# wmtlab/tactileSR

Hardware: AMD Instinct MI355X
Metric: SR samples/sec (4x4->40x40) (higher is better)
Workload: dtype f32 as 2 power-of-two-scaled fp16 planes x 3 MFMA products, fp32 accumulate (fp32-grade); 1 GPU; tactileSR_model eval forward 4x4->40x40, batch=4096/GPU, fp32 in/out (BASELINE configs[1]); batch_per_gpu=4096, scale_factor=10, seqsCnt=1, parallelism=replicas x1, conv_impl=fp16x3, dist_world_size=1

## Files before the change

### include/tactilesr_hip.h

```cpp
#ifndef TACTILESR_HIP_H
#define TACTILESR_HIP_H
#ifdef __cplusplus
extern "C" {
#endif

#define TSR_OK 0
#define TSR_ERR_ARG 1
#define TSR_ERR_LAUNCH 2

int tsr_abi_version(void);

int tsr_build_flags(void);

int tsr_pack_conv_weight(const float* w_oihw, float* w_packed, int cout, int cin, int ks, void* stream);

int tsr_conv2d_fwd(const float* in, int in_ctot, int in_coff, int cin,
                   const float* w_packed, int cout, int ks,
                   const float* scale, const float* shift,
                   const float* res, int res_ctot, int res_coff,
                   float* out, int out_ctot, int out_coff, int relu,
                   int B, int H, int W, void* stream);

long long tsr_conv_weight_bf16s_elems(int cout, int cin, int ks, int nsplit);
int tsr_pack_conv_weight_bf16s(const float* w_oihw, void* w_packed, int cout, int cin, int ks, int nsplit,
// ... 20 lines not shown
int tsr_conv2d_fwd_f16s(const float* in, int in_ctot, int in_coff, int cin,
                        const void* w_packed, int cout, int ks, float w_inv_scale,
                        const float* in_amax, float* out_amax,
                        const float* scale, const float* shift,
                        const float* res, int res_ctot, int res_coff,
                        float* out, int out_ctot, int out_coff, int relu,
                        int B, int H, int W, void* stream);
int tsr_conv2d_fwd_f16s_fuse1x1(const float* in, int in_ctot, int in_coff, int cin,
                                const void* w_packed, int ks, float w_inv_scale,
                                const float* in_amax, float* out_amax,
                                const float* scale, const float* shift, int relu,
                                const void* w2_packed, float w2_inv_scale, const float* shift2,
                                const float* res, int res_ctot, int res_coff,
                                float* out, int out_ctot, int out_coff, int relu2,
                                int B, int H, int W, void* stream);
int tsr_conv2d_fwd_b16(const void* in, int in_ctot, int in_coff, int cin, const void* w_packed, int cout, int ks,
                       const float* scale, const float* shift, const void* res, int res_ctot, int res_coff,
                       void* out, int out_ctot, int out_coff, int relu, int B, int H, int W, void* stream);
long long tsr_conv_weight_b16k_elems(int cout, int cin, int ks);
int tsr_pack_conv_weight_b16k(const float* w_oihw, void* w_packed, int cout, int cin, int ks, void* stream);
int tsr_pack_w2_b16k(const float* w2_64x128, void* w_packed, void* stream);
int tsr_conv2d_ex_dgrad_b16k(int nprime, int cout, int ks);
int tsr_conv2d_ex_fwd1x1_b16k(int cout, int cin);
int tsr_pack_conv_weight_dgrad_b16k(const float* w_oihw, void* w_packed, int cout, int cin, int ks, int ci0, int nprime,
                                    void* stream);
long long tsr_conv_weight_b16k_pair_elems(int cin);
int tsr_pack_conv_weight_b16k_pair(const float* w128_oihw5, void* w_packed, int cin, void* stream);
int tsr_conv2d_fwd_b16k(const void* in, int in_ctot, int in_coff, int cin, const void* w_packed, int cout, int ks,
                        const float* scale, const float* shift, const void* res, int res_ctot, int res_coff,
                        void* out, int out_ctot, int out_coff, int relu, int B, int H, int W, void* stream);
// ... 252 lines not shown
```

### tactilesr_amd/_lib.py

```python
from __future__ import annotations

import ctypes
import os
from ctypes import c_int, c_void_p, c_float, c_longlong, c_double

import torch

_HERE = os.path.dirname(os.path.abspath(__file__))
LIB_PATH = os.environ.get("TSR_LIB_OVERRIDE") or os.path.join(_HERE, "lib", "libtactilesr_hip.so")
ABI_VERSION = 24

_P, _I, _F, _L = c_void_p, c_int, c_float, c_longlong

SIGNATURES = {
    "tsr_abi_version": [],
    "tsr_build_flags": [],
    "tsr_pack_conv_weight": [_P, _P, _I, _I, _I, _P],
    "tsr_conv2d_fwd": [_P, _I, _I, _I, _P, _I, _I, _P, _P, _P, _I, _I, _P, _I, _I, _I, _I, _I, _I, _P],
    "tsr_conv_weight_bf16s_elems": [_I, _I, _I, _I],
    "tsr_pack_conv_weight_bf16s": [_P, _P, _I, _I, _I, _I, _P],
    "tsr_conv2d_fwd_bf16s": [_P, _I, _I, _I, _P, _I, _I, _I, _P, _P, _P, _I, _I, _P, _I, _I, _I, _I, _I, _I, _P],
    "tsr_stem_fwd": [_P, _I, _I, _I, _I, _I, _I, _P, _P, _P, _P, _I, _I, _I, _I, _P, _P],
    "tsr_pack_conv_weight_f16s": [_P, _P, _I, _I, _I, _F, _P],
    "tsr_pack_conv_weight_f16s_dev": [_P, _P, _I, _I, _I, _P, _P],
    "tsr_pack_conv_weight_dgrad_f16s_dev": [_P, _P, _I, _I, _I, _I, _I, _P, _P],
    "tsr_conv2d_fwd_f16s": [_P, _I, _I, _I, _P, _I, _I, _F, _P, _P, _P, _P, _P, _I, _I, _P, _I, _I, _I, _I, _I, _I, _P],
    "tsr_conv2d_fwd_f16s_fuse1x1": [_P, _I, _I, _I, _P, _I, _F, _P, _P, _P, _P, _I, _P, _F, _P, _P, _I, _I, _P, _I, _I,
                                    _I, _I, _I, _I, _P],
    "tsr_pair_channel_perm": [_P],
    "tsr_conv_weight_pair_elems": [_I],
    "tsr_pack_conv_weight_pair_f16s": [_P, _P, _P, _I, _F, _P, _P],
    "tsr_conv2d_fwd_f16s_pair": [_P, _I, _I, _I, _P, _F, _P, _P, _P, _P, _P, _I, _I, _I, _I, _I, _I, _P],
    "tsr_head_fwd": [_P, _I, _I, _P, _P, _I, _I, _I, _I, _P],
    "tsr_conv2d_fwd_b16": [_P, _I, _I, _I, _P, _I, _I, _P, _P, _P, _I, _I, _P, _I, _I, _I, _I, _I, _I, _P],
    "tsr_conv_weight_b16k_elems": [_I, _I, _I],
    "tsr_pack_conv_weight_b16k": [_P, _P, _I, _I, _I, _P],
    "tsr_pack_w2_b16k": [_P, _P, _P],
    "tsr_conv2d_ex_dgrad_b16k": [_I, _I, _I],
    "tsr_pack_conv_weight_dgrad_b16k": [_P, _P, _I, _I, _I, _I, _I, _P],
    "tsr_conv_weight_b16k_pair_elems": [_I],
    "tsr_pack_conv_weight_b16k_pair": [_P, _P, _I, _P],
    "tsr_conv2d_fwd_b16k": [_P, _I, _I, _I, _P, _I, _I, _P, _P, _P, _I, _I, _P, _I, _I, _I, _I, _I, _I, _P],
    "tsr_conv2d_fwd_b16k_fuse1x1": [_P, _I, _I, _I, _P, _I, _P, _P, _I, _P, _P, _P, _I, _I, _P, _I, _I, _I, _I, _I, _I, _P],
    "tsr_conv2d_fwd_b16k_pair": [_P, _I, _I, _I, _P, _P, _P, _P, _I, _I, _I, _I, _I, _I, _P],
    "tsr_stem_fwd_b16": [_P, _I, _I, _I, _I, _I, _I, _P, _P, _P, _P, _I, _I, _I, _I, _P],
    "tsr_head_fwd_b16": [_P, _I, _I, _P, _P, _I, _I, _I, _I, _P],
    "tsr_conv2d_ex": [_P, _P],
# ... 151 lines not shown
```

### tactilesr_amd/csrc/conv_args.h

```cpp
#pragma once
struct ConvArgs {
  const float* in;  int in_ctot;  int in_coff;  int cin;
  const float* wp;
  const float* scale; const float* shift;
  const float* res; int res_ctot; int res_coff;
  float* out; int out_ctot; int out_coff;
  int relu;
  int B, H, W;
  int tiles_x, tiles_y;
  const float* in_scale; const float* in_shift;
  const float* res_scale; const float* res_shift;
  int epi_mode;
  const float* mask; int mask_ctot; int mask_coff;
  const float* mask_scale; const float* mask_shift;
  const float* bn_a; const float* bn_b;
  float* slab; float* slab_cnt;
  const float* in_amax;
  float w_inv_scale;
  float* out_amax;
  const void* w2;
  float w2_inv_scale;
  const float* shift2;
  int relu2;
  const float* w_amax;
};
```

### tactilesr_amd/csrc/conv_epilogue16.h

```cpp
#pragma once
#include "tsr_common.h"
#include "conv_args.h"
#include "conv_epilogue.h"

template <int COUT, bool EXT, int WN = 2, bool IO16 = false>
__device__ __forceinline__ void conv_epilogue16(const ConvArgs& a, f32x4 (&acc)[4][COUT / (16 * WN)], int ebase, int b0,
                                                int y0, int x0, int wm, int wn, int lane, int HW, float accmul = 1.f) {
  constexpr int NT = COUT / (16 * WN);
  const int cl = lane & 15, ph = lane >> 4;
  const int k4 = cl >> 2, j = cl & 3;
  const int dyl = ph >> 1, dxl = 4 * (ph & 1);
  float amax = 0.f;
  const int b = b0 + wm;
  const bool img_ok = b < a.B;
  const int out_blocks = a.out_ctot >> 4;
  const int res_blocks = a.res_ctot >> 4;
  const int mask_blocks = a.mask_ctot >> 4;
  const int bsafe = img_ok ? b : 0;
  typedef __bf16 ep_bf16x4 __attribute__((ext_vector_type(4)));
  const int gx = x0 + dxl + j;
  const f32x4 one4v = {1.f, 1.f, 1.f, 1.f}, zero4v = {0.f, 0.f, 0.f, 0.f};
  f32x4 pv0[NT], pv1[NT], pv2[NT], pv3[NT], pv4[NT];
  const bool m2 = EXT && a.epi_mode == 2, m0 = !EXT || a.epi_mode == 0;
#pragma unroll
// ... 54 lines not shown
          for (int c = 0; c < 4; ++c) v[c] = (v[c] * accmul) * sc4[c] + sh4[c];
          if (rb4) {
            f32x4 rv = rvv[mt];
            if (EXT && a.res_scale) {
#pragma unroll
              for (int c = 0; c < 4; ++c) rv[c] = tsr_relu(fmaf(rv[c], rsc4[c], rsh4[c]));
            }
#pragma unroll
            for (int c = 0; c < 4; ++c) v[c] += rv[c];
          }
#pragma unroll
          for (int c = 0; c < 4; ++c) {
            if (a.relu) v[c] = tsr_relu(v[c]);
            amax = fmaxf(amax, fabsf(v[c]));
          }
          if (IO16) {
            ep_bf16x4 o16;
#pragma unroll
            for (int c = 0; c < 4; ++c) o16[c] = (__bf16)v[c];
            *(ep_bf16x4*)((__bf16*)a.out + oidx4 + po) = o16;
          } else {
            *(f32x4*)(ob4 + po) = v;
          }
        }
      }
    } else if (EXT && a.epi_mode == 1) {
      float cnt = 0.f, sum = 0.f;
#pragma unroll
      for (int mt = 0; mt < 4; ++mt) {
#pragma unroll
        for (int r = 0; r < 4; ++r) {
// ... 83 lines not shown
        for (int c = 0; c < 4; ++c) {
          s1[c] += __shfl_xor(s1[c], 1); s2[c] += __shfl_xor(s2[c], 1);
          s1[c] += __shfl_xor(s1[c], 2); s2[c] += __shfl_xor(s2[c], 2);
          s1[c] += __shfl_xor(s1[c], 16); s2[c] += __shfl_xor(s2[c], 16);
          s1[c] += __shfl_xor(s1[c], 32); s2[c] += __shfl_xor(s2[c], 32);
        }
        if (ph == 0 && j == 0) {
          const size_t e = (size_t)ebase + wm;
          float* sl = a.slab + (e * COUT + nq) * 2;
#pragma unroll
          for (int c = 0; c < 4; ++c) { sl[2 * c] = s1[c]; sl[2 * c + 1] = s2[c]; }
        }
      }
    }
  }
  if (a.out_amax) {
#pragma unroll
    for (int o = 32; o > 0; o >>= 1) amax = fmaxf(amax, __shfl_xor(amax, o));
    if (lane == 0) publish_amax(a.out_amax, amax);
  }
}
```

### tactilesr_amd/csrc/conv_mfma_k32.hip

```cpp
#include "tsr_common.h"
#include "conv_args.h"
#include "conv_epilogue16.h"
#include "conv_fuse1x1_16.h"
#include "conv_host.h"
#include "tactilesr_hip.h"
#include <type_traits>

typedef _Float16 kf16x8 __attribute__((ext_vector_type(8)));
typedef _Float16 kf16x4 __attribute__((ext_vector_type(4)));

constexpr int k32_row_slots(int px) {
  int rs = px * 4;
  while ((rs & 3) != 2) ++rs;
  return rs;
}

template <int KS, int COUT, int WN, bool DBH = false, int NTHR = 256> struct K32Geom {
  static constexpr int IMG = (NTHR / 64) / WN;
  static constexpr int HH = 8 + KS - 1;
  static constexpr int T = KS * KS;
  static constexpr int HS = (T - 1) / 2;
  static constexpr int PIXB = 64;
  static constexpr int ROWB = k32_row_slots(HH) * 16;
  static constexpr int IMGB = HH * ROWB;
  static constexpr int HALO_B = IMG * IMGB;
  static constexpr int SROWB = k32_row_slots(8) * 16;
  static constexpr int SIMGB = 8 * SROWB;
  static constexpr int SIDE_B = DBH ? 0 : IMG * SIMGB;
  static constexpr int WTAP_B = 2 * 16 * COUT * 2;
  static constexpr int WSLAB_B = 2 * WTAP_B;
  static constexpr int NHB = DBH ? 2 : 1;
  static constexpr int MAIN_LDS = NHB * HALO_B + SIDE_B + 3 * WSLAB_B;
};

constexpr int PAIR_KH[12] = {0, 0, 0, 2, 1, 3, 4, 4, 1, 1, 2, 3};
constexpr int PAIR_KW[12] = {0, 2, 4, 4, 0, 0, 1, 3, 1, 3, 1, 1};
constexpr int PAIR_V[12] = {0, 0, 1, 1, 1, 1, 0, 0, 0, 1, 0, 0};
constexpr int PAIR_OUTER = 8;

template <int KS, int COUT, bool EXT, int WN, bool FUSE2 = false, bool DBH = false, int NTHR = 256, bool PAIR = false>
__global__ __launch_bounds__(NTHR, NTHR == 512 ? 1 : 2) void conv_k32_kernel(const ConvArgs a) {
  static_assert(!PAIR || (KS == 5 && COUT == 128 && !EXT && !FUSE2 && !DBH), "pair form: 5x5 geometry, inference");
  static_assert(COUT == 64 * WN, "every wave owns 64 channels");
  static_assert(!FUSE2 || (!EXT && COUT == 128), "fused 1x1: 128 channels, inference");
  static_assert(NTHR == 256 || (NTHR == 512 && WN == 2), "512 threads: 4 images x 2 C_out halves");
  typedef K32Geom<KS, COUT, WN, DBH, NTHR> G;
  constexpr int NW = NTHR / 64;
  constexpr bool WDMA = !EXT;
  constexpr int IMG = G::IMG, P = KS / 2, HH = G::HH, T = G::T, HS = G::HS, NT = COUT / (16 * WN);
  constexpr int PIXB = G::PIXB, ROWB = G::ROWB, IMGB = G::IMGB, HALO_B = G::HALO_B;
  constexpr int SROWB = G::SROWB, SIMGB = G::SIMGB, SIDE_B = G::SIDE_B;
  constexpr int WTAP_B = G::WTAP_B, WSLAB_B = G::WSLAB_B;
  constexpr int WITEMS = WSLAB_B / 16, WV = (WITEMS + NTHR - 1) / NTHR;
  constexpr int NITEM = IMG * HH * HH * 4, NIT = (NITEM + NTHR - 1) / NTHR;
  constexpr int FUSE_LDS = FUSE2 ? Fuse1x1Geom16<IMG>::BYTES + 64 : 0;
  __shared__ __attribute__((aligned(16))) char lds[G::MAIN_LDS > FUSE_LDS ? G::MAIN_LDS : FUSE_LDS];
  char* halo = lds;
  char* wbuf = lds + G::NHB * HALO_B + SIDE_B;

  const int tid = threadIdx.x;
  const int lane = tid & 63;
  const int wave = tid >> 6;
  const int wave_s = __builtin_amdgcn_readfirstlane(wave);
  const int wm = WN == 2 ? wave >> 1 : wave, wn = WN == 2 ? wave & 1 : 0;
  const int m = lane & 15, g = lane >> 4, khalf = g & 1, tsel = g >> 1;

  float sx = 1.f, accmul = 1.f, sxh = 1.f;
  int bid;
  {
    const int nwg = gridDim.x, q = nwg >> 3, r = nwg & 7;
    const int xcd = blockIdx.x & 7, idx = blockIdx.x >> 3;
    bid = (xcd < r ? xcd * (q + 1) : r * (q + 1) + (xcd - r) * q) + idx;
  }
  const int tpi = a.tiles_x * a.tiles_y;
  const int ig = bid / tpi;
  const int trem = bid - ig * tpi;
  const int ebase = bid * IMG;
  const int ty = trem / a.tiles_x, tx = trem - ty * a.tiles_x;
  const int y0 = ty * 8, x0 = tx * 8, b0 = ig * IMG;
  const int HW = a.H * a.W;
  const int in_blocks = a.in_ctot >> 4;

  int st_src[NIT], st_dst[NIT];
#pragma unroll
  for (int k = 0; k < NIT; ++k) {
    const int it = tid + k * NTHR;
    st_src[k] = -1;
    st_dst[k] = -1;
    if (it < NITEM) {
      const int qd = it & 3, px = it >> 2;
      const int img = px / (HH * HH), rem = px - img * (HH * HH);
      const int hy = rem / HH, hx = rem - hy * HH;
      const int gy = y0 - P + hy, gx = x0 - P + hx, b = b0 + img;
      st_dst[k] = img * IMGB + hy * ROWB + hx * PIXB + qd * 8;
      if (b < a.B && gy >= 0 && gy < a.H && gx >= 0 && gx < a.W)
        st_src[k] = ((img * in_blocks) * HW + gy * a.W + gx) * 16 + qd * 4;
    }
  }
  const float* in_base = a.in + ((size_t)b0 * in_blocks + (a.in_coff >> 4)) * HW * 16;

  const int laneA0 = wm * IMGB + (m >> 3) * ROWB + (m & 7) * PIXB + khalf * 16;
  const int lx = laneA0 + tsel * PIXB;
  constexpr int CK = PAIR ? 3 : KS - 1;
  const int lw = PAIR ? laneA0 + tsel * ROWB
                      : laneA0 + tsel * (ROWB - (KS - 1) * PIXB);
  const int lc = tsel ? laneA0 + CK * ROWB + CK * PIXB
                      : HALO_B + wm * SIMGB + (m >> 3) * SROWB + (m & 7) * PIXB + khalf * 16;
  const int lcs = tsel ? 2 * ROWB : 2 * SROWB;
  const int lcd = laneA0 + (KS - 1) * (ROWB + PIXB) + tsel * HALO_B;
// ... 15 lines not shown

  f32x4 hsc = {1.f, 1.f, 1.f, 1.f}, hsh = {0.f, 0.f, 0.f, 0.f};
  auto load_halo = [&](int c, f32x4* hv) __attribute__((always_inline)) {
    const float* inc = in_base + (size_t)(c < nreal ? c : nreal - 1) * HW * 16;
    if (EXT && a.in_scale) {
      const int cq = (c < nreal ? c : nreal - 1) * 16 + (tid & 3) * 4;
      hsc = *(const f32x4*)(a.in_scale + cq);
      hsh = *(const f32x4*)(a.in_shift + cq);
    }
#pragma unroll
    for (int k = 0; k < NIT; ++k) hv[k] = *(const f32x4*)(inc + (unsigned)(st_src[k] < 0 ? 0 : st_src[k]));
  };
  auto store_halo = [&](const f32x4* hv, int c, int hb = 0) __attribute__((always_inline)) {
#pragma unroll
    for (int k = 0; k < NIT; ++k) {
      if (st_dst[k] >= 0) {
        f32x4 v = hv[k];
        if (EXT && a.in_scale) {
#pragma unroll
          for (int jj = 0; jj < 4; ++jj) v[jj] = tsr_relu_x2(fmaf(v[jj], hsc[jj], hsh[jj]));
        }
        const bool inside = st_src[k] >= 0 && c < nreal;
#pragma unroll
        for (int jj = 0; jj < 4; ++jj) v[jj] = inside ? v[jj] * sxh : 0.f;
#pragma unroll
        for (int p = 0; p < 2; ++p) {
          kf16x4 bq;
#pragma unroll
          for (int jj = 0; jj < 4; ++jj) {
            bq[jj] = (_Float16)v[jj];
            v[jj] -= (float)bq[jj];
          }
          *(kf16x4*)(halo + hb * HALO_B + st_dst[k] + p * 32) = bq;
        }
      }
    }
  };
#define DMA_BYTES(goff_, slot_, nv_)                                                     \
  {                                                                                      \
    const int vo_ = (int)(goff_) + tid * 16;                                             \
    char* dst_ = wbuf + (slot_) * WSLAB_B + wave_s * 1024;                               \
    _Pragma("unroll") for (int v = 0; v < (nv_); ++v)                                    \
      __builtin_amdgcn_raw_ptr_buffer_load_lds(wrsrc, (__attribute__((address_space(3))) void*)(dst_ + v * NTHR * 16), 16, \
                                               vo_ + v * NTHR * 16, 0, 0, 0);             \
  }
#define DMA_PIECE(vo_, slot_, v_)                                                        \
  __builtin_amdgcn_raw_ptr_buffer_load_lds(wrsrc, (__attribute__((address_space(3))) void*)(wbuf + (slot_) * WSLAB_B + wave_s * 1024 + (v_) * NTHR * 16), \
                                           16, (vo_) + (v_) * NTHR * 16, 0, 0, 0)
#define LOAD_W(sidx)                                                                     \
  {                                                                                      \
// ... 74 lines not shown
      __builtin_amdgcn_sched_group_barrier(0x100, 1, 0);                                 \
    } else if ((nr_) == 1) {                                                             \
      __builtin_amdgcn_sched_group_barrier(0x008, (nm_), 0);                             \
      __builtin_amdgcn_sched_group_barrier(0x100, 1, 0);                                 \
    } else {                                                                             \
      __builtin_amdgcn_sched_group_barrier(0x008, (nm_), 0);                             \
    }                                                                                    \
    if (pc_) __builtin_amdgcn_sched_group_barrier(0x040, 1, 0);                          \
    __builtin_amdgcn_sched_barrier(0);                                                   \
  }
  constexpr bool WROWS = WDMA && KS == 5 && !PAIR;
#define PIECE_AT(g_) if ((g_) < WV) DMA_PIECE(vo, slot2, (g_))

  auto operand_scales = [&]() __attribute__((always_inline)) {
    float mx = a.in_amax ? *a.in_amax : 0.f;
    if (EXT && a.in_scale) {
      __shared__ float bnd[2 * NW];
      float ms = 0.f, mt = 0.f;
      for (int c = threadIdx.x; c < a.cin; c += NTHR) {
        ms = fmaxf(ms, fabsf(a.in_scale[c]));
        mt = fmaxf(mt, fabsf(a.in_shift[c]));
      }
#pragma unroll
      for (int o = 32; o > 0; o >>= 1) {
        ms = fmaxf(ms, __shfl_xor(ms, o));
        mt = fmaxf(mt, __shfl_xor(mt, o));
      }
      if (lane == 0) { bnd[wave * 2] = ms; bnd[wave * 2 + 1] = mt; }
      __syncthreads();
      ms = 0.f; mt = 0.f;
#pragma unroll
      for (int w = 0; w < NW; ++w) { ms = fmaxf(ms, bnd[2 * w]); mt = fmaxf(mt, bnd[2 * w + 1]); }
      mx = mx * ms + mt;
    }
    if (mx > 0.f) {
      int e = (int)((__float_as_uint(mx) >> 23) & 0xFF) - 127;
      int be = 13 - e + 127;
      be = be < 1 ? 1 : (be > 254 ? 254 : be);
      sx = __uint_as_float((unsigned)be << 23);
    }
    float w_inv = a.w_inv_scale;
    if (a.w_amax) {
      const float wmx = *a.w_amax;
      w_inv = 1.f;
      if (wmx > 0.f && wmx < 3.0e38f) {
        int be = 127 - (13 - ((int)((__float_as_uint(wmx) >> 23) & 0xFF) - 127));
        be = be < 1 ? 1 : (be > 254 ? 254 : be);
        w_inv = __uint_as_float((unsigned)be << 23);
      }
    }
    accmul = w_inv / sx;
    sxh = (EXT && a.in_scale) ? 0.5f * sx : sx;
  };

  f32x4 hv[NIT], wreg[WDMA ? 1 : WV];
  size_t woff = 0;
  load_halo(0, hv);
  if constexpr (PAIR) {
    DMA_WP(0, 0);
    DMA_WP(1, 1);
    operand_scales();
  } else if constexpr (WDMA) {
    DMA_W(0, 0);
    if (S > 1) DMA_W(1, 1);
    operand_scales();
  } else {
    LOAD_W(0);
    operand_scales();
    STORE_W(0);
    if (S > 1) { LOAD_W(1); STORE_W(1); }
  }
  store_halo(hv, 0);
  if constexpr (WDMA) { DMA_WAIT(); } else { if (S > 2) LOAD_W(2); }
  __syncthreads();

  kf16x8 A0[4], A1[4], B0[NT] = {}, B1[NT] = {};
  LOAD_A(A1, 1, 0, 0);
  if constexpr (PAIR) { LOAD_B_HI(B0, 0, 0); } else { LOAD_B(B0, 0, 0); }

  constexpr int SCI = IMG * 256 / NTHR, SCS = NTHR / 256;
  const int sc_t = tid & 255, sc_i0 = tid >> 8;
  const int sc_src = sc_i0 * IMGB + ((sc_t >> 5) + CK) * ROWB + (((sc_t >> 2) & 7) + CK) * PIXB + (sc_t & 3) * 16;
  const int sc_dst = HALO_B + sc_i0 * SIMGB + (sc_t >> 5) * SROWB + ((sc_t >> 2) & 7) * PIXB + (sc_t & 3) * 16;

  int s = 0;
  int slot = 0;
  auto block = [&](int c, auto oddc) __attribute__((always_inline)) {
// ... 108 lines not shown
      slot = slot1;
    }
  };
  if constexpr (!DBH) {
    for (int c = 0; c < nchunk; c += 2) {
      block(c, std::integral_constant<int, 0>());
      block(c + 1, std::integral_constant<int, 1>());
    }
  } else {
    for (int c = 0; c < nchunk; c += 2) {
#pragma unroll
      for (int p = 0; p < T; ++p) {
        const int slot1 = slot == 2 ? 0 : slot + 1;
        const int slot2 = slot1 == 2 ? 0 : slot1 + 1;
        if (WDMA && s + 2 < S) DMA_W(s + 2, slot2);
        if (p == HS) { LOAD_A_CROSSD(A0, 0); }
        else if (p < HS) { LOAD_A(A0, 0, p, 0); }
        else { LOAD_A(A0, 0, p - HS - 1, 1); }
        LOAD_B(B1, 1, slot);
        if (p == 0) load_halo(c + 1, hv);
        if (p == HS + 1 && c + 2 < nchunk) load_halo(c + 2, hv);
        MFMA_PHASE(A1, B0);
        INTERLEAVE(8, 2);
        if (p + 1 == HS) { LOAD_A_CROSSD(A1, 1); }
        else if (p + 1 < HS) { LOAD_A(A1, 1, p + 1, 0); }
        else if (p + 1 < T) { LOAD_A(A1, 1, p - HS, 1); }
        else { LOAD_A(A1, 1, 0, 0); }
        MFMA_PHASE(A0, B0);
        INTERLEAVE(4, 4);
        LOAD_B(B0, 0, slot1);
        MFMA_PHASE(A0, B1);
        INTERLEAVE(4, 4);
        if (p == HS - 2) store_halo(hv, c + 1, 1);
        if (p == T - 2 && c + 2 < nchunk) store_halo(hv, c + 2, 0);
        if constexpr (WDMA) {
          if (p == 0 || (p == HS + 1 && c + 2 < nchunk)) { DMA_WAIT_N(NIT); } else { DMA_WAIT(); }
        } else {
          if (s + 2 < S) STORE_W(slot2);
          if (s + 3 < S) LOAD_W(s + 3);
        }
        STEP_BARRIER();
        ++s;
        slot = slot1;
      }
    }
  }
#undef DMA_W
#undef LOAD_W
#undef STORE_W
#undef DMA_WP
#undef DMA_BYTES
// ... 8 lines not shown
#undef LOAD_B_HI
#undef MFMA_PHASE_HI
#undef MFMA_PHASE
#undef INTERLEAVE
#undef MFMA_ROW
#undef HINT_ROW
#undef PIECE_AT
#undef DMA_PIECE
#undef LOAD_A_1
#undef LOAD_A_CROSS_1
#undef LOAD_A_CROSSD_1
#undef LOAD_B_1
#undef LOAD_B_HI_1

  if constexpr (FUSE2) conv_fuse1x1_epilogue16<IMG>(a, acc, lds, b0, y0, x0, wm, wn, lane, HW, accmul);
  else conv_epilogue16<COUT, EXT, WN>(a, acc, ebase, b0, y0, x0, wm, wn, lane, HW, accmul);
}

int tsr_conv_k32_images(int cout) { (void)cout; return 4; }

template <int KS, int COUT, bool EXT>
static int launch_k32(const ConvArgs& a, hipStream_t st) {
  constexpr int WN = COUT / 64;
  if constexpr (COUT == 128 && EXT) {
    const int grid = ((a.B + 3) / 4) * a.tiles_x * a.tiles_y;
    hipLaunchKernelGGL((conv_k32_kernel<KS, COUT, EXT, WN, false, KS == 3, 512>), dim3(grid), dim3(512), 0, st, a);
    return tsr_check_launch();
  }
  constexpr int IMG = 4 / WN;
  const int grid = ((a.B + IMG - 1) / IMG) * a.tiles_x * a.tiles_y;
  hipLaunchKernelGGL((conv_k32_kernel<KS, COUT, EXT, WN, false, KS == 3>), dim3(grid), dim3(256), 0, st, a);
// ... 91 lines not shown
      conv_fill(a, in, in_ctot, in_coff, cin, w_packed, scale, shift, nullptr, 0, 0, out, out_ctot, out_coff, 128, relu, B, H, W))
    return TSR_ERR_ARG;
  a.in_amax = in_amax; a.w_inv_scale = w_inv_scale; a.out_amax = out_amax;
  const int grid = ((B + 1) / 2) * a.tiles_x * a.tiles_y;
  hipLaunchKernelGGL((conv_k32_kernel<5, 128, false, 2, false, false, 256, true>), dim3(grid), dim3(256), 0,
                     (hipStream_t)stream, a);
  return tsr_check_launch();
}

int tsr_conv_k32_fuse1x1(const ConvArgs& a, int ks, hipStream_t st) {
  const int grid = ((a.B + 1) / 2) * a.tiles_x * a.tiles_y;
  if (ks == 5) hipLaunchKernelGGL((conv_k32_kernel<5, 128, false, 2, true>), dim3(grid), dim3(256), 0, st, a);
  else hipLaunchKernelGGL((conv_k32_kernel<3, 128, false, 2, true, true>), dim3(grid), dim3(256), 0, st, a);
  return tsr_check_launch();
}
```

### tactilesr_amd/model/tactileSR_model.py

```python
from __future__ import annotations

import math
from typing import Dict, Optional

import torch
import torch.nn as nn

from .. import _lib
from .._lib import call, ptr, stream

_I = _lib.c_int


def _conv_bn_relu(cin: int, cout: int, k: int, bias: bool) -> nn.Sequential:
    return nn.Sequential(nn.Conv2d(cin, cout, k, padding=k // 2, bias=bias), nn.BatchNorm2d(cout), nn.ReLU(True))


def _reference_init(root: nn.Module) -> None:
    for m in root.modules():
        if isinstance(m, nn.Conv2d):
            nn.init.kaiming_normal_(m.weight, mode="fan_out", nonlinearity="relu")
        elif isinstance(m, nn.BatchNorm2d):
            nn.init.constant_(m.weight, 0.1)
            nn.init.constant_(m.bias, 0.1)
# ... 245 lines not shown

    def __init__(self, conv: nn.Conv2d, bn: Optional[nn.BatchNorm2d], nsplit: int = 0, cin_perm=None):
        w = conv.weight.detach().float()
        if cin_perm is not None:
            w = w[:, cin_perm]
        w = w.contiguous()
        self.cout, self.cin, self.ks = w.shape[0], w.shape[1], w.shape[2]
        self.nsplit = nsplit
        self.io16 = nsplit == CONV_IMPLS["bf16"]
        self.b16k = self.io16 and self.ks > 1 and self.cin % 32 == 0 and self.cout == 128
        self.w, self.w_inv_scale = _pack_host(w, NS_B16K if self.b16k else nsplit)
        self.scale, self.shift = _fold(conv.bias, bn, self.cout, w.device)


class _PackedPair:
    __slots__ = ("w", "scale", "shift", "cin", "w_inv_scale", "perm")
    b16k = False
    _perm = None

    @classmethod
    def channel_perm(cls, device):
        if cls._perm is None:
            import ctypes
            arr = (ctypes.c_int * 128)()
            call("tsr_pair_channel_perm", ctypes.cast(arr, ctypes.c_void_p))
            cls._perm = list(arr)
        return torch.tensor(cls._perm, dtype=torch.long, device=device)

    def __init__(self, seq3: nn.Sequential, seq5: nn.Sequential):
        w3 = seq3[0].weight.detach().float().contiguous()
        w5 = seq5[0].weight.detach().float().contiguous()
        self.cin = w3.shape[1]
        wscale = _pow2_wscale(max(float(w3.abs().max()), float(w5.abs().max())))
        self.w_inv_scale = 1.0 / wscale
        self.w = torch.empty(_lib.load().tsr_conv_weight_pair_elems(self.cin), dtype=torch.float16, device=w3.device)
        call("tsr_pack_conv_weight_pair_f16s", ptr(w3), ptr(w5), ptr(self.w), _I(self.cin), _lib.c_float(wscale),
             ptr(None), stream())
        s3, sh3 = _fold(seq3[0].bias, seq3[1], 64, w3.device)
        s5, sh5 = _fold(seq5[0].bias, seq5[1], 64, w3.device)
        self.perm = self.channel_perm(w3.device)
        self.scale = torch.cat([s3, s5])[self.perm].contiguous()
        self.shift = torch.cat([sh3, sh5])[self.perm].contiguous()


class _PackedPairB16:
    __slots__ = ("w", "scale", "shift", "cin")
    b16k = True
    perm = None

    def __init__(self, seq3: nn.Sequential, seq5: nn.Sequential):
        w3 = seq3[0].weight.detach().float()
        w5 = seq5[0].weight.detach().float()
        self.cin = w3.shape[1]
        self.w = _pack_pair_b16k(w3, w5)
        s3, sh3 = _fold(seq3[0].bias, seq3[1], 64, w3.device)
        s5, sh5 = _fold(seq5[0].bias, seq5[1], 64, w3.device)
        self.scale = torch.cat([s3, s5]).contiguous()
# ... 13 lines not shown
        self.w, self.w_inv_scale = _pack_host(w, NS_F16X3)


def _fold(bias, bn: Optional[nn.BatchNorm2d], cout: int, device):
    if bn is None:
        if bias is None:
            return None, None
        return None, bias.detach().float().contiguous()
    scale = bn.weight.detach().float() / torch.sqrt(bn.running_var.detach().float() + bn.eps)
    b = bias.detach().float() if bias is not None else torch.zeros(cout, device=device)
    shift = (b - bn.running_mean.detach().float()) * scale + bn.bias.detach().float()
    return scale.contiguous(), shift.contiguous()


class _MSRBPlan:
    __slots__ = ("pair", "c31", "c51", "c32", "c52", "conf", "halves")


class _ResPlan:
    __slots__ = ("c1", "c2")


def _msrb_plan(blk, ns, fuse_pair, fuse_1x1, bf16_storage) -> _MSRBPlan:
    p = _MSRBPlan()
    has_fused = ns == NS_F16X3 or bf16_storage
    p.halves = p.pair = p.c31 = p.c51 = None
    if fuse_1x1 and has_fused:
        p.halves = tuple(_PackedHalf(blk.confusion.weight.detach()[:, o:o + 128], ns) for o in (0, 128))
    if fuse_pair and has_fused:
        p.pair = (_PackedPairB16 if bf16_storage else _PackedPair)(blk.conv_3_1, blk.conv_5_1)
    else:
        p.c31 = _PackedConv(blk.conv_3_1[0], blk.conv_3_1[1], ns)
        p.c51 = _PackedConv(blk.conv_5_1[0], blk.conv_5_1[1], ns)
    perm = p.pair.perm if p.pair is not None else None
    p.c32 = _PackedConv(blk.conv_3_2[0], blk.conv_3_2[1], ns, cin_perm=perm)
    p.c52 = _PackedConv(blk.conv_5_2[0], blk.conv_5_2[1], ns, cin_perm=perm)
    p.conf = _PackedConv(blk.confusion, None, ns)
    return p


def _res_plan(rb, ns) -> _ResPlan:
    p = _ResPlan()
    p.c1, p.c2 = _PackedConv(rb.conv1, None, ns), _PackedConv(rb.conv2, None, ns)
    return p


def _conv(prof, pc: _PackedConv, src, s_ctot, s_coff, dst, d_ctot, d_coff, relu, B, H, W, res=None, r_ctot=0, r_coff=0,
          amax_in=None, amax_out=None):
    with _timed(prof, (pc.ks, pc.cout)):
# ... 4 lines not shown
        elif pc.nsplit == NS_F16X3:
            call("tsr_conv2d_fwd_f16s", ptr(src), _I(s_ctot), _I(s_coff), _I(pc.cin), ptr(pc.w), _I(pc.cout),
                 _I(pc.ks), _lib.c_float(pc.w_inv_scale), ptr(amax_in), ptr(amax_out), ptr(pc.scale), ptr(pc.shift),
                 ptr(res), _I(r_ctot), _I(r_coff), ptr(dst), _I(d_ctot), _I(d_coff), _I(1 if relu else 0),
                 _I(B), _I(H), _I(W), stream())
        elif pc.nsplit == NS_F32:
            call("tsr_conv2d_fwd", ptr(src), _I(s_ctot), _I(s_coff), _I(pc.cin), ptr(pc.w), _I(pc.cout), _I(pc.ks),
                 ptr(pc.scale), ptr(pc.shift), ptr(res), _I(r_ctot), _I(r_coff),
                 ptr(dst), _I(d_ctot), _I(d_coff), _I(1 if relu else 0), _I(B), _I(H), _I(W), stream())
        else:
            call("tsr_conv2d_fwd_bf16s", ptr(src), _I(s_ctot), _I(s_coff), _I(pc.cin), ptr(pc.w), _I(pc.cout),
                 _I(pc.ks), _I(pc.nsplit), ptr(pc.scale), ptr(pc.shift), ptr(res), _I(r_ctot), _I(r_coff),
                 ptr(dst), _I(d_ctot), _I(d_coff), _I(1 if relu else 0), _I(B), _I(H), _I(W), stream())


def _conv_pair(prof, pp, src, dst, B, H, W, amax_in, amax_out):
    with _timed(prof, ("pair", 128)):
        if pp.b16k:
            call("tsr_conv2d_fwd_b16k_pair", ptr(src), _I(64), _I(0), _I(pp.cin), ptr(pp.w), ptr(pp.scale), ptr(pp.shift),
                 ptr(dst), _I(128), _I(0), _I(1), _I(B), _I(H), _I(W), stream())
        else:
            call("tsr_conv2d_fwd_f16s_pair", ptr(src), _I(64), _I(0), _I(pp.cin), ptr(pp.w), _lib.c_float(pp.w_inv_scale),
                 ptr(amax_in), ptr(amax_out), ptr(pp.scale), ptr(pp.shift), ptr(dst), _I(128), _I(0), _I(1),
                 _I(B), _I(H), _I(W), stream())


def _conv_fused(prof, pc: _PackedConv, half: _PackedHalf, shift2, src, dst, d_ctot, d_coff, res, r_ctot, r_coff, relu2,
                amax_out, amax_in, B, H, W):
    with _timed(prof, (pc.ks, pc.cout)):
        if pc.io16:
            call("tsr_conv2d_fwd_b16k_fuse1x1", ptr(src), _I(128), _I(0), _I(128), ptr(pc.w), _I(pc.ks), ptr(pc.scale),
                 ptr(pc.shift), _I(1), ptr(half.w), ptr(shift2), ptr(res), _I(r_ctot), _I(r_coff), ptr(dst), _I(d_ctot),
                 _I(d_coff), _I(1 if relu2 else 0), _I(B), _I(H), _I(W), stream())
        else:
            call("tsr_conv2d_fwd_f16s_fuse1x1", ptr(src), _I(128), _I(0), _I(128), ptr(pc.w), _I(pc.ks),
                 _lib.c_float(pc.w_inv_scale), ptr(amax_in), ptr(amax_out), ptr(pc.scale), ptr(pc.shift), _I(1),
                 ptr(half.w), _lib.c_float(half.w_inv_scale), ptr(shift2), ptr(res), _I(r_ctot), _I(r_coff),
                 ptr(dst), _I(d_ctot), _I(d_coff), _I(1 if relu2 else 0), _I(B), _I(H), _I(W), stream())


def _msrb_workspace(fused: bool, like: torch.Tensor, BHW: int):
    return like.new_empty(128 * BHW), like.new_empty((64 if fused else 256) * BHW)


def _run_msrb(p: _MSRBPlan, prof, src, s_in, dst, d_ctot, d_coff, s_out, ws, slot, B, H, W):
    cat1, ws2 = ws
    s_c1, s_c2 = slot(), slot()
    if p.pair is not None:
        _conv_pair(prof, p.pair, src, cat1, B, H, W, s_in, s_c1)
    else:
        _conv(prof, p.c31, src, 64, 0, cat1, 128, 0, True, B, H, W, amax_in=s_in, amax_out=s_c1)
        _conv(prof, p.c51, src, 64, 0, cat1, 128, 64, True, B, H, W, amax_in=s_in, amax_out=s_c1)
    if p.halves is not None:
        _conv_fused(prof, p.c32, p.halves[0], p.conf.shift, cat1, ws2, 64, 0, src, 64, 0, False, None, s_c1, B, H, W)
        _conv_fused(prof, p.c52, p.halves[1], None, cat1, dst, d_ctot, d_coff, ws2, 64, 0, True, s_out, s_c1, B, H, W)
    else:
        _conv(prof, p.c32, cat1, 128, 0, ws2, 256, 0, True, B, H, W, amax_in=s_c1, amax_out=s_c2)
        _conv(prof, p.c52, cat1, 128, 0, ws2, 256, 128, True, B, H, W, amax_in=s_c1, amax_out=s_c2)
        _conv(prof, p.conf, ws2, 256, 0, dst, d_ctot, d_coff, True, B, H, W, res=src, r_ctot=64, r_coff=0,
              amax_in=s_c2, amax_out=s_out)


# ... 327 lines not shown
```

Before: 31020 samples/s.

## Store MSRB cat1 pre-split as fp16 hi/lo planes with analytic scale bound

The pair conv now writes its output already split into two fp16 planes. It scales them with a power-of-two factor derived from an analytic bound: the input amax times the weight/BN gain, plus the max shift. That bound replaces the measured output amax. The fused 1x1 consumers load the pre-split halo directly, through raw copies or buffer_load-to-LDS DMA for the 3x3 double-buffered form, so they skip the fp32-to-fp16x2 conversion and do not depend on an amax reduction. The intent is to cut conversion ALU work and register-staged halo traffic. The cost is a looser scale bound, which may lose fp16 precision headroom, plus inline-asm DMA complexity.

```diff
diff --git a/include/tactilesr_hip.h b/include/tactilesr_hip.h
--- a/include/tactilesr_hip.h
+++ b/include/tactilesr_hip.h
@@ -58,6 +58,16 @@
                                 const float* res, int res_ctot, int res_coff,
                                 float* out, int out_ctot, int out_coff, int relu2,
                                 int B, int H, int W, void* stream);
+int tsr_conv2d_fwd_f16s_pair_split(const float* in, int in_ctot, int in_coff, int cin, const void* w_packed,
+                                   float w_inv_scale, const float* in_amax, float bound_g, float bound_d,
+                                   const float* scale, const float* shift, void* out, int out_ctot, int out_coff,
+                                   int relu, int B, int H, int W, void* stream);
+int tsr_conv2d_fwd_f16s_fuse1x1_split(const void* in, int in_ctot, int in_coff, int cin, const void* w_packed, int ks,
+                                      float w_inv_scale, const float* src_amax, float bound_g, float bound_d,
+                                      float* out_amax, const float* scale, const float* shift, int relu,
+                                      const void* w2_packed, float w2_inv_scale, const float* shift2,
+                                      const float* res, int res_ctot, int res_coff, float* out, int out_ctot,
+                                      int out_coff, int relu2, int B, int H, int W, void* stream);
 int tsr_conv2d_fwd_b16(const void* in, int in_ctot, int in_coff, int cin, const void* w_packed, int cout, int ks,
                        const float* scale, const float* shift, const void* res, int res_ctot, int res_coff,
                        void* out, int out_ctot, int out_coff, int relu, int B, int H, int W, void* stream);
diff --git a/tactilesr_amd/_lib.py b/tactilesr_amd/_lib.py
--- a/tactilesr_amd/_lib.py
+++ b/tactilesr_amd/_lib.py
@@ -31,6 +31,9 @@
     "tsr_conv_weight_pair_elems": [_I],
     "tsr_pack_conv_weight_pair_f16s": [_P, _P, _P, _I, _F, _P, _P],
     "tsr_conv2d_fwd_f16s_pair": [_P, _I, _I, _I, _P, _F, _P, _P, _P, _P, _P, _I, _I, _I, _I, _I, _I, _P],
+    "tsr_conv2d_fwd_f16s_pair_split": [_P, _I, _I, _I, _P, _F, _P, _F, _F, _P, _P, _P, _I, _I, _I, _I, _I, _I, _P],
+    "tsr_conv2d_fwd_f16s_fuse1x1_split": [_P, _I, _I, _I, _P, _I, _F, _P, _F, _F, _P, _P, _P, _I, _P, _F, _P, _P, _I, _I, _P,
+                                          _I, _I, _I, _I, _I, _I, _P],
     "tsr_head_fwd": [_P, _I, _I, _P, _P, _I, _I, _I, _I, _P],
     "tsr_conv2d_fwd_b16": [_P, _I, _I, _I, _P, _I, _I, _P, _P, _P, _I, _I, _P, _I, _I, _I, _I, _I, _I, _P],
     "tsr_conv_weight_b16k_elems": [_I, _I, _I],
diff --git a/tactilesr_amd/csrc/conv_args.h b/tactilesr_amd/csrc/conv_args.h
--- a/tactilesr_amd/csrc/conv_args.h
+++ b/tactilesr_amd/csrc/conv_args.h
@@ -23,4 +23,17 @@
   const float* shift2;
   int relu2;
   const float* w_amax;
+  const float* src_amax;
+  float bound_g, bound_d;
 };
+
+#if defined(__HIPCC__)
+__device__ __forceinline__ float f16s_split_bound(float src_amax, float g, float d) { return __builtin_fmaf(src_amax, g, d); }
+__device__ __forceinline__ float f16s_pow2_scale(float mx) {
+  if (!(mx > 0.f)) return 1.f;
+  const int e = (int)((__builtin_bit_cast(unsigned, mx) >> 23) & 0xFF) - 127;
+  int be = 13 - e + 127;
+  be = be < 1 ? 1 : (be > 254 ? 254 : be);
+  return __builtin_bit_cast(float, (unsigned)be << 23);
+}
+#endif
diff --git a/tactilesr_amd/csrc/conv_epilogue16.h b/tactilesr_amd/csrc/conv_epilogue16.h
--- a/tactilesr_amd/csrc/conv_epilogue16.h
+++ b/tactilesr_amd/csrc/conv_epilogue16.h
@@ -3,9 +3,11 @@
 #include "conv_args.h"
 #include "conv_epilogue.h"
 
-template <int COUT, bool EXT, int WN = 2, bool IO16 = false>
+template <int COUT, bool EXT, int WN = 2, bool IO16 = false, bool SPLIT = false>
 __device__ __forceinline__ void conv_epilogue16(const ConvArgs& a, f32x4 (&acc)[4][COUT / (16 * WN)], int ebase, int b0,
-                                                int y0, int x0, int wm, int wn, int lane, int HW, float accmul = 1.f) {
+                                                int y0, int x0, int wm, int wn, int lane, int HW, float accmul = 1.f,
+                                                float sx_out = 1.f) {
+  static_assert(!SPLIT || (!EXT && !IO16), "pre-split output: inference, fp32-sized elements");
   constexpr int NT = COUT / (16 * WN);
   const int cl = lane & 15, ph = lane >> 4;
   const int k4 = cl >> 2, j = cl & 3;
@@ -92,7 +94,19 @@
             if (a.relu) v[c] = tsr_relu(v[c]);
             amax = fmaxf(amax, fabsf(v[c]));
           }
-          if (IO16) {
+          if (SPLIT) {
+            typedef _Float16 ep_f16x4 __attribute__((ext_vector_type(4)));
+            ep_f16x4 h1, h2;
+#pragma unroll
+            for (int c = 0; c < 4; ++c) {
+              const float vs = v[c] * sx_out;
+              h1[c] = (_Float16)vs;
+              h2[c] = (_Float16)(vs - (float)h1[c]);
+            }
+            char* ob = (char*)(a.out + oidx4 - (oq & 15) + po) + (oq & 15) * 2;
+            *(ep_f16x4*)ob = h1;
+            *(ep_f16x4*)(ob + 32) = h2;
+          } else if (IO16) {
             ep_bf16x4 o16;
 #pragma unroll
             for (int c = 0; c < 4; ++c) o16[c] = (__bf16)v[c];
@@ -206,7 +220,7 @@
       }
     }
   }
-  if (a.out_amax) {
+  if (!SPLIT && a.out_amax) {
 #pragma unroll
     for (int o = 32; o > 0; o >>= 1) amax = fmaxf(amax, __shfl_xor(amax, o));
     if (lane == 0) publish_amax(a.out_amax, amax);
diff --git a/tactilesr_amd/csrc/conv_mfma_k32.hip b/tactilesr_amd/csrc/conv_mfma_k32.hip
--- a/tactilesr_amd/csrc/conv_mfma_k32.hip
+++ b/tactilesr_amd/csrc/conv_mfma_k32.hip
@@ -33,14 +33,26 @@
   static constexpr int MAIN_LDS = NHB * HALO_B + SIDE_B + 3 * WSLAB_B;
 };
 
+typedef int ki32x4 __attribute__((ext_vector_type(4)));
+__device__ __forceinline__ void k32_dma_row(ki32x4 rs, int vo, int so, unsigned m0v, unsigned long long mask) {
+  unsigned long long sv;
+  unsigned keep;
+  asm volatile("s_mov_b32 %1, m0\n\ts_mov_b64 %0, exec\n\ts_mov_b64 exec, %6\n\ts_mov_b32 m0, %2\n\ts_nop 0\n\t"
+               "buffer_load_dwordx4 %3, %4, %5 offen lds\n\ts_mov_b64 exec, %0\n\ts_mov_b32 m0, %1"
+               : "=&s"(sv), "=&s"(keep) : "s"(m0v), "v"(vo), "s"(rs), "s"(so), "s"(mask) : "memory");
+}
+
 constexpr int PAIR_KH[12] = {0, 0, 0, 2, 1, 3, 4, 4, 1, 1, 2, 3};
 constexpr int PAIR_KW[12] = {0, 2, 4, 4, 0, 0, 1, 3, 1, 3, 1, 1};
 constexpr int PAIR_V[12] = {0, 0, 1, 1, 1, 1, 0, 0, 0, 1, 0, 0};
 constexpr int PAIR_OUTER = 8;
 
-template <int KS, int COUT, bool EXT, int WN, bool FUSE2 = false, bool DBH = false, int NTHR = 256, bool PAIR = false>
+template <int KS, int COUT, bool EXT, int WN, bool FUSE2 = false, bool DBH = false, int NTHR = 256, bool PAIR = false,
+          bool SPLIT = false>
 __global__ __launch_bounds__(NTHR, NTHR == 512 ? 1 : 2) void conv_k32_kernel(const ConvArgs a) {
   static_assert(!PAIR || (KS == 5 && COUT == 128 && !EXT && !FUSE2 && !DBH), "pair form: 5x5 geometry, inference");
+  static_assert(!SPLIT || ((PAIR || FUSE2) && NTHR == 256), "split cat1: written by the pair form, read by the fused forms");
+  constexpr bool SPLIT_IN = SPLIT && FUSE2, SPLIT_OUT = SPLIT && PAIR;
   static_assert(COUT == 64 * WN, "every wave owns 64 channels");
   static_assert(!FUSE2 || (!EXT && COUT == 128), "fused 1x1: 128 channels, inference");
   static_assert(NTHR == 256 || (NTHR == 512 && WN == 2), "512 threads: 4 images x 2 C_out halves");
@@ -66,6 +78,7 @@
   const int m = lane & 15, g = lane >> 4, khalf = g & 1, tsel = g >> 1;
 
   float sx = 1.f, accmul = 1.f, sxh = 1.f;
+  float sx_out = 1.f;
   int bid;
   {
     const int nwg = gridDim.x, q = nwg >> 3, r = nwg & 7;
@@ -92,7 +105,7 @@
       const int img = px / (HH * HH), rem = px - img * (HH * HH);
       const int hy = rem / HH, hx = rem - hy * HH;
       const int gy = y0 - P + hy, gx = x0 - P + hx, b = b0 + img;
-      st_dst[k] = img * IMGB + hy * ROWB + hx * PIXB + qd * 8;
+      st_dst[k] = img * IMGB + hy * ROWB + hx * PIXB + qd * (SPLIT_IN ? 16 : 8);
       if (b < a.B && gy >= 0 && gy < a.H && gx >= 0 && gx < a.W)
         st_src[k] = ((img * in_blocks) * HW + gy * a.W + gx) * 16 + qd * 4;
     }
@@ -138,7 +151,14 @@
   auto store_halo = [&](const f32x4* hv, int c, int hb = 0) __attribute__((always_inline)) {
 #pragma unroll
     for (int k = 0; k < NIT; ++k) {
-      if (st_dst[k] >= 0) {
+      if (SPLIT_IN) {
+        if (st_dst[k] >= 0) {
+          typedef int ki32x4 __attribute__((ext_vector_type(4)));
+          const bool inside = st_src[k] >= 0 && c < nreal;
+          const ki32x4 raw = __builtin_bit_cast(ki32x4, hv[k]);
+          *(ki32x4*)(halo + hb * HALO_B + st_dst[k]) = inside ? raw : (ki32x4){0, 0, 0, 0};
+        }
+      } else if (st_dst[k] >= 0) {
         f32x4 v = hv[k];
         if (EXT && a.in_scale) {
 #pragma unroll
@@ -158,6 +178,25 @@
           *(kf16x4*)(halo + hb * HALO_B + st_dst[k] + p * 32) = bq;
         }
       }
+    }
+  };
+  constexpr bool HDMA = SPLIT_IN && DBH;
+  constexpr int RPW = IMG * HH / NW;
+  static_assert(!HDMA || (IMG * HH % NW == 0 && HH % RPW == 0 && HH * 4 <= 64), "whole rows per wave, one image per wave");
+  const int hd_img = (wave_s * RPW) / HH, hd_r0 = (wave_s * RPW) % HH;
+  const int hd_gx = x0 - P + (lane >> 2);
+  const int hd_vo = ((lane >> 2) < HH && hd_gx >= 0 && hd_gx < a.W && b0 + hd_img < a.B) ? hd_gx * 64 + (lane & 3) * 16
+                                                                                         : (int)0x80000000;
+  const unsigned long long hd_base = (unsigned long long)(const char*)in_base;
+  const unsigned hd_lds = (unsigned)(size_t)(const __attribute__((address_space(3))) char*)halo + hd_img * IMGB + hd_r0 * ROWB;
+  auto dma_halo = [&](int c, int hb) __attribute__((always_inline)) {
+#pragma unroll
+    for (int k = 0; k < RPW; ++k) {
+      const int gy = y0 - P + hd_r0 + k;
+      const bool row_ok = c < nreal && gy >= 0 && gy < a.H;
+      const ki32x4 rs = {(int)hd_base, (int)(hd_base >> 32) & 0xffff, 0x7fffffff & -(int)row_ok, 0x00020000};
+      const int so = (((hd_img * in_blocks + c) * HW + gy * a.W) * 64) & -(int)row_ok;
+      k32_dma_row(rs, hd_vo, so, hd_lds + hb * HALO_B + k * ROWB, (1ull << (4 * HH)) - 1);
     }
   };
 #define DMA_BYTES(goff_, slot_, nv_)                                                     \
@@ -262,6 +301,8 @@
 
   auto operand_scales = [&]() __attribute__((always_inline)) {
     float mx = a.in_amax ? *a.in_amax : 0.f;
+    if (SPLIT_IN) mx = f16s_split_bound(*a.src_amax, a.bound_g, a.bound_d);
+    if (SPLIT_OUT) sx_out = f16s_pow2_scale(f16s_split_bound(mx, a.bound_g, a.bound_d));
     if (EXT && a.in_scale) {
       __shared__ float bnd[2 * NW];
       float ms = 0.f, mt = 0.f;
@@ -281,12 +322,7 @@
       for (int w = 0; w < NW; ++w) { ms = fmaxf(ms, bnd[2 * w]); mt = fmaxf(mt, bnd[2 * w + 1]); }
       mx = mx * ms + mt;
     }
-    if (mx > 0.f) {
-      int e = (int)((__float_as_uint(mx) >> 23) & 0xFF) - 127;
-      int be = 13 - e + 127;
-      be = be < 1 ? 1 : (be > 254 ? 254 : be);
-      sx = __uint_as_float((unsigned)be << 23);
-    }
+    sx = f16s_pow2_scale(mx);
     float w_inv = a.w_inv_scale;
     if (a.w_amax) {
       const float wmx = *a.w_amax;
@@ -303,7 +339,8 @@
 
   f32x4 hv[NIT], wreg[WDMA ? 1 : WV];
   size_t woff = 0;
-  load_halo(0, hv);
+  (void)dma_halo;
+  if constexpr (HDMA) dma_halo(0, 0); else load_halo(0, hv);
   if constexpr (PAIR) {
     DMA_WP(0, 0);
     DMA_WP(1, 1);
@@ -318,7 +355,7 @@
     STORE_W(0);
     if (S > 1) { LOAD_W(1); STORE_W(1); }
   }
-  store_halo(hv, 0);
+  if constexpr (!HDMA) store_halo(hv, 0);
   if constexpr (WDMA) { DMA_WAIT(); } else { if (S > 2) LOAD_W(2); }
   __syncthreads();
 
@@ -457,12 +494,18 @@
         const int slot1 = slot == 2 ? 0 : slot + 1;
         const int slot2 = slot1 == 2 ? 0 : slot1 + 1;
         if (WDMA && s + 2 < S) DMA_W(s + 2, slot2);
+        if constexpr (HDMA) {
+          if (p == 0) dma_halo(c + 1, 1);
+          if (p == HS + 1 && c + 2 < nchunk) dma_halo(c + 2, 0);
+        }
         if (p == HS) { LOAD_A_CROSSD(A0, 0); }
         else if (p < HS) { LOAD_A(A0, 0, p, 0); }
         else { LOAD_A(A0, 0, p - HS - 1, 1); }
         LOAD_B(B1, 1, slot);
-        if (p == 0) load_halo(c + 1, hv);
-        if (p == HS + 1 && c + 2 < nchunk) load_halo(c + 2, hv);
+        if constexpr (!HDMA) {
+          if (p == 0) load_halo(c + 1, hv);
+          if (p == HS + 1 && c + 2 < nchunk) load_halo(c + 2, hv);
+        }
         MFMA_PHASE(A1, B0);
         INTERLEAVE(8, 2);
         if (p + 1 == HS) { LOAD_A_CROSSD(A1, 1); }
@@ -474,10 +517,12 @@
         LOAD_B(B0, 0, slot1);
         MFMA_PHASE(A0, B1);
         INTERLEAVE(4, 4);
-        if (p == HS - 2) store_halo(hv, c + 1, 1);
-        if (p == T - 2 && c + 2 < nchunk) store_halo(hv, c + 2, 0);
+        if constexpr (!HDMA) {
+          if (p == HS - 2) store_halo(hv, c + 1, 1);
+          if (p == T - 2 && c + 2 < nchunk) store_halo(hv, c + 2, 0);
+        }
         if constexpr (WDMA) {
-          if (p == 0 || (p == HS + 1 && c + 2 < nchunk)) { DMA_WAIT_N(NIT); } else { DMA_WAIT(); }
+          if (p == 0 || (p == HS + 1 && c + 2 < nchunk)) { DMA_WAIT_N(HDMA ? RPW : NIT); } else { DMA_WAIT(); }
         } else {
           if (s + 2 < S) STORE_W(slot2);
           if (s + 3 < S) LOAD_W(s + 3);
@@ -516,7 +561,7 @@
 #undef LOAD_B_HI_1
 
   if constexpr (FUSE2) conv_fuse1x1_epilogue16<IMG>(a, acc, lds, b0, y0, x0, wm, wn, lane, HW, accmul);
-  else conv_epilogue16<COUT, EXT, WN>(a, acc, ebase, b0, y0, x0, wm, wn, lane, HW, accmul);
+  else conv_epilogue16<COUT, EXT, WN, false, SPLIT_OUT>(a, acc, ebase, b0, y0, x0, wm, wn, lane, HW, accmul, sx_out);
 }
 
 int tsr_conv_k32_images(int cout) { (void)cout; return 4; }
@@ -638,3 +683,43 @@
   else hipLaunchKernelGGL((conv_k32_kernel<3, 128, false, 2, true, true>), dim3(grid), dim3(256), 0, st, a);
   return tsr_check_launch();
 }
+
+static inline bool split_bound_ok(float g, float d) { return g >= 0.f && d >= 0.f && g < 3.0e38f && d < 3.0e38f; }
+
+extern "C" int tsr_conv2d_fwd_f16s_pair_split(const float* in, int in_ctot, int in_coff, int cin, const void* w_packed,
+                                              float w_inv_scale, const float* in_amax, float bound_g, float bound_d,
+                                              const float* scale, const float* shift, void* out, int out_ctot, int out_coff,
+                                              int relu, int B, int H, int W, void* stream) {
+  ConvArgs a;
+  if (!f16s_scales_ok(in_amax, w_inv_scale) || !split_bound_ok(bound_g, bound_d) ||
+      conv_fill(a, in, in_ctot, in_coff, cin, w_packed, scale, shift, nullptr, 0, 0, out, out_ctot, out_coff, 128, relu, B, H, W))
+    return TSR_ERR_ARG;
+  a.in_amax = in_amax; a.w_inv_scale = w_inv_scale;
+  a.bound_g = bound_g; a.bound_d = bound_d;
+  const int grid = ((B + 1) / 2) * a.tiles_x * a.tiles_y;
+  hipLaunchKernelGGL((conv_k32_kernel<5, 128, false, 2, false, false, 256, true, true>), dim3(grid), dim3(256), 0,
+                     (hipStream_t)stream, a);
+  return tsr_check_launch();
+}
+
+extern "C" int tsr_conv2d_fwd_f16s_fuse1x1_split(const void* in, int in_ctot, int in_coff, int cin, const void* w_packed, int ks,
+                                                 float w_inv_scale, const float* src_amax, float bound_g, float bound_d,
+                                                 float* out_amax, const float* scale, const float* shift, int relu,
+                                                 const void* w2_packed, float w2_inv_scale, const float* shift2,
+                                                 const float* res, int res_ctot, int res_coff, float* out, int out_ctot,
+                                                 int out_coff, int relu2, int B, int H, int W, void* stream) {
+  ConvArgs a;
+  if (!f16s_scales_ok(src_amax, w_inv_scale) || !split_bound_ok(bound_g, bound_d) || !w2_packed || !(w2_inv_scale > 0.f) ||
+      (ks != 3 && ks != 5) || (cin & 31) ||
+      conv_fill(a, in, in_ctot, in_coff, cin, w_packed, scale, shift, res, res_ctot, res_coff, out, out_ctot, out_coff, 64, relu,
+                B, H, W))
+    return TSR_ERR_ARG;
+  a.src_amax = src_amax; a.bound_g = bound_g; a.bound_d = bound_d;
+  a.w_inv_scale = w_inv_scale; a.out_amax = out_amax;
+  a.w2 = w2_packed; a.w2_inv_scale = w2_inv_scale; a.shift2 = shift2; a.relu2 = relu2;
+  const int grid = ((B + 1) / 2) * a.tiles_x * a.tiles_y;
+  hipStream_t st = (hipStream_t)stream;
+  if (ks == 5) hipLaunchKernelGGL((conv_k32_kernel<5, 128, false, 2, true, false, 256, false, true>), dim3(grid), dim3(256), 0, st, a);
+  else hipLaunchKernelGGL((conv_k32_kernel<3, 128, false, 2, true, true, 256, false, true>), dim3(grid), dim3(256), 0, st, a);
+  return tsr_check_launch();
+}
diff --git a/tactilesr_amd/model/tactileSR_model.py b/tactilesr_amd/model/tactileSR_model.py
--- a/tactilesr_amd/model/tactileSR_model.py
+++ b/tactilesr_amd/model/tactileSR_model.py
@@ -283,7 +283,7 @@
 
 
 class _PackedPair:
-    __slots__ = ("w", "scale", "shift", "cin", "w_inv_scale", "perm")
+    __slots__ = ("w", "scale", "shift", "cin", "w_inv_scale", "perm", "bound_g", "bound_d")
     b16k = False
     _perm = None
 
@@ -310,6 +310,10 @@
         self.perm = self.channel_perm(w3.device)
         self.scale = torch.cat([s3, s5])[self.perm].contiguous()
         self.shift = torch.cat([sh3, sh5])[self.perm].contiguous()
+        gain = torch.cat([w3.double().abs().sum((1, 2, 3)) * s3.double().abs(),
+                          w5.double().abs().sum((1, 2, 3)) * s5.double().abs()]).max()
+        self.bound_g = float(torch.nextafter(gain.float().cpu(), torch.tensor(math.inf)))
+        self.bound_d = max(0.0, float(self.shift.max()))
 
 
 class _PackedPairB16:
@@ -353,7 +357,7 @@
 
 
 class _MSRBPlan:
-    __slots__ = ("pair", "c31", "c51", "c32", "c52", "conf", "halves")
+    __slots__ = ("pair", "c31", "c51", "c32", "c52", "conf", "halves", "split")
 
 
 class _ResPlan:
@@ -372,6 +376,7 @@
         p.c31 = _PackedConv(blk.conv_3_1[0], blk.conv_3_1[1], ns)
         p.c51 = _PackedConv(blk.conv_5_1[0], blk.conv_5_1[1], ns)
     perm = p.pair.perm if p.pair is not None else None
+    p.split = p.pair is not None and p.halves is not None and not bf16_storage
     p.c32 = _PackedConv(blk.conv_3_2[0], blk.conv_3_2[1], ns, cin_perm=perm)
     p.c52 = _PackedConv(blk.conv_5_2[0], blk.conv_5_2[1], ns, cin_perm=perm)
     p.conf = _PackedConv(blk.confusion, None, ns)
@@ -406,11 +411,15 @@
                  ptr(dst), _I(d_ctot), _I(d_coff), _I(1 if relu else 0), _I(B), _I(H), _I(W), stream())
 
 
-def _conv_pair(prof, pp, src, dst, B, H, W, amax_in, amax_out):
+def _conv_pair(prof, pp, src, dst, B, H, W, amax_in, amax_out, split=False):
     with _timed(prof, ("pair", 128)):
         if pp.b16k:
             call("tsr_conv2d_fwd_b16k_pair", ptr(src), _I(64), _I(0), _I(pp.cin), ptr(pp.w), ptr(pp.scale), ptr(pp.shift),
                  ptr(dst), _I(128), _I(0), _I(1), _I(B), _I(H), _I(W), stream())
+        elif split:
+            call("tsr_conv2d_fwd_f16s_pair_split", ptr(src), _I(64), _I(0), _I(pp.cin), ptr(pp.w),
+                 _lib.c_float(pp.w_inv_scale), ptr(amax_in), _lib.c_float(pp.bound_g), _lib.c_float(pp.bound_d),
+                 ptr(pp.scale), ptr(pp.shift), ptr(dst), _I(128), _I(0), _I(1), _I(B), _I(H), _I(W), stream())
         else:
             call("tsr_conv2d_fwd_f16s_pair", ptr(src), _I(64), _I(0), _I(pp.cin), ptr(pp.w), _lib.c_float(pp.w_inv_scale),
                  ptr(amax_in), ptr(amax_out), ptr(pp.scale), ptr(pp.shift), ptr(dst), _I(128), _I(0), _I(1),
@@ -418,12 +427,18 @@
 
 
 def _conv_fused(prof, pc: _PackedConv, half: _PackedHalf, shift2, src, dst, d_ctot, d_coff, res, r_ctot, r_coff, relu2,
-                amax_out, amax_in, B, H, W):
+                amax_out, amax_in, B, H, W, split=None):
     with _timed(prof, (pc.ks, pc.cout)):
         if pc.io16:
             call("tsr_conv2d_fwd_b16k_fuse1x1", ptr(src), _I(128), _I(0), _I(128), ptr(pc.w), _I(pc.ks), ptr(pc.scale),
                  ptr(pc.shift), _I(1), ptr(half.w), ptr(shift2), ptr(res), _I(r_ctot), _I(r_coff), ptr(dst), _I(d_ctot),
                  _I(d_coff), _I(1 if relu2 else 0), _I(B), _I(H), _I(W), stream())
+        elif split is not None:
+            call("tsr_conv2d_fwd_f16s_fuse1x1_split", ptr(src), _I(128), _I(0), _I(128), ptr(pc.w), _I(pc.ks),
+                 _lib.c_float(pc.w_inv_scale), ptr(amax_in), _lib.c_float(split.bound_g), _lib.c_float(split.bound_d),
+                 ptr(amax_out), ptr(pc.scale), ptr(pc.shift), _I(1), ptr(half.w), _lib.c_float(half.w_inv_scale),
+                 ptr(shift2), ptr(res), _I(r_ctot), _I(r_coff), ptr(dst), _I(d_ctot), _I(d_coff), _I(1 if relu2 else 0),
+                 _I(B), _I(H), _I(W), stream())
         else:
             call("tsr_conv2d_fwd_f16s_fuse1x1", ptr(src), _I(128), _I(0), _I(128), ptr(pc.w), _I(pc.ks),
                  _lib.c_float(pc.w_inv_scale), ptr(amax_in), ptr(amax_out), ptr(pc.scale), ptr(pc.shift), _I(1),
@@ -438,6 +453,13 @@
 def _run_msrb(p: _MSRBPlan, prof, src, s_in, dst, d_ctot, d_coff, s_out, ws, slot, B, H, W):
     cat1, ws2 = ws
     s_c1, s_c2 = slot(), slot()
+    if p.split:
+        _conv_pair(prof, p.pair, src, cat1, B, H, W, s_in, None, split=True)
+        _conv_fused(prof, p.c32, p.halves[0], p.conf.shift, cat1, ws2, 64, 0, src, 64, 0, False, None, s_in, B, H, W,
+                    split=p.pair)
+        _conv_fused(prof, p.c52, p.halves[1], None, cat1, dst, d_ctot, d_coff, ws2, 64, 0, True, s_out, s_in, B, H, W,
+                    split=p.pair)
+        return
     if p.pair is not None:
         _conv_pair(prof, p.pair, src, cat1, B, H, W, s_in, s_c1)
     else:
```

Measured after the change: 31280 samples/s (median of 6 runs). No clear change (+0.8%).
